# highreso-gpu/k8s-watcher

Measured on AMD Instinct MI355X. Metric: pod-events/sec sustained + p50 event→notify latency (single process, mock API), higher is better.
Workload: dtype n/a; 1 GPU; global_batch=1600000, parallelism=single-process (cluster watch), api_server=http, clusterapi=http, namespaces=64, target_namespaces=32, engine=native, validate=payload, state_format=structured

## Files before the change

### k8s_watcher_amd/ops/csrc/check/chunked_check.cpp

```cpp

#include <algorithm>
#include <cstdint>
#include <cstdio>
#include <cstdlib>
#include <cstring>
#include <fstream>
#include <iostream>
#include <memory>
#include <string>
#include <string_view>
#include <vector>

#if defined(__x86_64__)
#include <immintrin.h>
#endif

namespace {

#include "../scanner.inc"
#include "../chunked.inc"

struct Out {
    std::vector<std::string> lines;
    std::string end;
    bool operator==(const Out& o) const { return lines == o.lines && end == o.end; }
};

bool blank(const char* b, size_t n) {
    for (size_t i = 0; i < n; ++i)
        if (!(b[i] == ' ' || b[i] == '\r' || b[i] == '\t' || b[i] == '\n')) return false;
    return true;
}

std::string final_state(const ChunkState& st, bool open) {
    if (st.done()) return "done";
    return "state " + std::to_string(st.cstate) + " remain " + std::to_string(st.cremain) + " open " +
           std::to_string((int)open);
}

bool keep(Out& out, const char* b, size_t n) {
    if (n && !blank(b, n)) out.lines.emplace_back(b, n);
    return true;
}
// ... 116 lines not shown
```

### k8s_watcher_amd/ops/csrc/chunked.inc

```

enum { CS_SIZE, CS_DATA, CS_DATA_END, CS_TRAILER, CS_DONE };

bool parse_chunk_size(const char* line, size_t n, size_t& size, bool lenient) {
    size_t v = 0;
    size_t i = 0;
    while (lenient && i < n && (line[i] == ' ' || line[i] == '\t')) ++i;
    size_t start = i;
    for (; i < n; ++i) {
        int h = hexval(line[i]);
        if (h < 0) break;
        if (v > (SIZE_MAX >> 4)) return false;
        v = (v << 4) | (size_t)h;
    }
    if (i == start) return false;
    while (i < n && (line[i] == ' ' || line[i] == '\t' || (lenient && line[i] == '\r'))) ++i;
    if (i < n && line[i] != ';') return false;
    size = v;
    return true;
}

bool parse_chunk_size(const std::string& line, size_t& size) {
    return parse_chunk_size(line.data(), line.size(), size, true);
}

struct ChunkState {
    int cstate = CS_SIZE;
    size_t cremain = 0;
    std::string line;
    bool done() const { return cstate == CS_DONE; }
};

enum ChunkEnd {
    CE_MORE,
    CE_STOPPED,
    CE_DONE,
    CE_TOO_LONG,
    CE_BAD_SIZE,
};

constexpr size_t CHUNK_LINE_MAX = 4096;

std::string chunk_error_text(const ChunkState& st, ChunkEnd e) {
    if (e == CE_TOO_LONG) return "chunk size line too long";
    char msg[64];
    std::snprintf(msg, sizeof msg, "bad chunk size line %.40s", st.line.c_str());
    return msg;
}

template <class Sink>
inline ChunkEnd chunk_deframe(ChunkState& st, const char* base, size_t from, size_t to, size_t& at, Sink&& sink) {
    size_t i = from;
    ChunkEnd end = CE_MORE;
    while (i < to && end == CE_MORE) {
        switch (st.cstate) {
            case CS_SIZE: {
                const char* nl = (const char*)std::memchr(base + i, '\n', to - i);
                if (!nl) {
                    st.line.append(base + i, to - i);
                    i = to;
                    if (st.line.size() > CHUNK_LINE_MAX) end = CE_TOO_LONG;
                    break;
                }
                st.line.append(base + i, (size_t)(nl - (base + i)));
                i = (size_t)(nl - base) + 1;
                size_t size;
                if (!parse_chunk_size(st.line, size)) {
                    end = CE_BAD_SIZE;
                    break;
                }
                st.line.clear();
                if (size == 0) {
                    st.cstate = CS_TRAILER;
                } else {
                    st.cremain = size;
                    st.cstate = CS_DATA;
                }
                break;
            }
            case CS_DATA: {
                const size_t take = st.cremain < to - i ? st.cremain : to - i;
                if (!sink(i, take)) end = CE_STOPPED;
                i += take;
                st.cremain -= take;
                if (st.cremain == 0) st.cstate = CS_DATA_END;
                break;
            }
            case CS_DATA_END: {
                const char* nl = (const char*)std::memchr(base + i, '\n', to - i);
                if (!nl) {
                    i = to;
                    break;
                }
                i = (size_t)(nl - base) + 1;
                st.cstate = CS_SIZE;
                break;
            }
            case CS_TRAILER: {
                const char* nl = (const char*)std::memchr(base + i, '\n', to - i);
                if (!nl) {
                    st.line.append(base + i, to - i);
                    i = to;
                    break;
                }
                st.line.append(base + i, (size_t)(nl - (base + i)));
                i = (size_t)(nl - base) + 1;
                const bool empty = st.line.empty() || (st.line.size() == 1 && st.line[0] == '\r');
                st.line.clear();
                if (empty) {
                    st.cstate = CS_DONE;
                    end = CE_DONE;
                }
                break;
            }
            default:
                end = CE_DONE;
        }
    }
    at = i;
    return end;
}

enum : uint8_t {
    LN_WHOLE = 0,
    LN_FRAG = 1,
    LN_FRAG_END = 2,
};

template <class Sink>
inline bool split_lines(const char* base, size_t a, size_t n, bool& open, Sink&& sink) {
    size_t pos = a;
    const size_t end = a + n;
    while (pos < end) {
        const char* nl = (const char*)std::memchr(base + pos, '\n', end - pos);
        if (!nl) {
            open = true;
            return sink(LN_FRAG, pos, end - pos);
        }
        const size_t len = (size_t)(nl - base) - pos;
        const uint8_t kind = open ? LN_FRAG_END : LN_WHOLE;
        open = false;
        pos += len + 1;
        if (!sink(kind, pos - len - 1, len)) return false;
    }
    return true;
}

template <class Line>
inline bool join_line(std::string& partial, uint8_t kind, const char* b, size_t n, Line&& line) {
    if (kind == LN_WHOLE) return line(b, n, (std::string*)nullptr);
    partial.append(b, n);
    if (kind == LN_FRAG) return true;
    const bool go = line(partial.data(), partial.size(), &partial);
    partial.clear();
    return go;
}
```

### k8s_watcher_amd/ops/csrc/engine.inc

```


struct NReq {
    uint64_t seq = 0;
    std::string uid, etype, ns, name, body;
    size_t nbytes = 0;
    int64_t read_ns = 0, sent_ns = 0;
    int64_t submit_ns = 0;
    int attempts = 0;
    int conn = 0;
};

struct NConn {
    int fd = -1;
    bool up = false;
    std::deque<uint64_t> queue, inflight;
    std::string out;
    size_t out_off = 0;
    std::string in;
    bool dirty = false;
    SSL* ssl = nullptr;
    bool handshaking = false;
    bool write_wants_read = false;
    struct Staged {
        const char* p;
// ... 24 lines not shown
        ERR_error_string_n(e, buf, sizeof buf);
        msg += ": ";
        msg += buf;
    }
    ERR_clear_error();
    return msg;
}

int64_t mono_ns() {
    struct timespec ts;
    clock_gettime(CLOCK_MONOTONIC, &ts);
    return (int64_t)ts.tv_sec * 1000000000LL + ts.tv_nsec;
}

struct Probe {
    bool on = false;
    int64_t t0_ns = 0;
    uint64_t t0_tsc = 0;
    uint64_t calls = 0, lines = 0, bytes = 0, split = 0, wait = 0, apply = 0, run = 0, nio_calls = 0, nio = 0;
    uint64_t pump = 0;
    uint64_t tail = 0;
    uint64_t partitioned = 0;
    uint64_t tail_serial = 0;
    uint64_t tail_sent = 0, tail_submit = 0;
    uint64_t tail_rv = 0;
    long double age_byte_ns = 0;
};
Probe g_probe;

struct ApplyStats {
    std::atomic<uint64_t> par_batches{0}, par_lines{0}, tail_serial{0}, tail_submits{0}, tail_lock_runs{0};
    std::atomic<uint64_t> serial_batches{0}, serial_lines{0};
    std::atomic<uint64_t> payload_built{0}, payload_prefiltered{0};
};
ApplyStats g_apply;

uint32_t crc32_bytes(const char* p, size_t n) {
    return (uint32_t)::crc32(0L, reinterpret_cast<const Bytef*>(p), (uInt)n);
}

struct NotifierCore {
    std::recursive_mutex mu;
    bool threaded = false;
    int ep = -1, wake_fd = -1, py_fd = -1;
    std::thread io;
    std::atomic<bool> io_quit{false};
    std::vector<uint8_t> epout;
    int64_t signal_below = -1;
    int64_t signal_below_bytes = -1;

    std::vector<NConn> conns;
    using ReqMap = std::unordered_map<uint64_t, NReq>;
    ReqMap reqs;
    SvMap<uint64_t> latest;
    SvMap<uint64_t> unsent;
    std::vector<ReqMap::node_type> free_reqs;
    std::vector<SvMap<uint64_t>::node_type> free_latest;
    static constexpr size_t FREE_NODES_MAX = 4096;
    std::string head;
    int depth = 1;
    int max_attempts = 3;
    double delay = 2.0, multiplier = 2.0, max_delay = 30.0;
    bool coalesce = false, log_events = false;
    LogSink* sink = nullptr;
    std::vector<int> retryable;
    uint64_t next_seq = 0;
// ... 1422 lines not shown
    const std::string* env_json;
    int extra = 0;
    uint8_t validate = VALIDATE_PAYLOAD;
    const std::string* tz_utc = nullptr;
    bool failures = false;
    const ReasonSet* reasons = nullptr;
    bool conditions = false;
    const CondRules* rules = nullptr;
};

enum : uint8_t {
    JOB_FULL = 0,
    JOB_FIELDS = 1,
    JOB_PAYLOAD = 2,
    JOB_SKIP = 3,
};

struct ApplyHot {
    Span uid, ns, name, rv, phase;
    size_t uid_h = 0, ns_h = 0;
    const char* err = nullptr;
    const char* payload_err = nullptr;
    int tidx = -1;
    bool status_present = false, uid_hashed = false, ns_hashed = false;
    bool has_core = false, repr_fallback = false, obj_present = false;
    bool fail_cand = false;
    bool cond_cand = false;
    bool pre_dropped = false;
    uint8_t part = 255;
    uint8_t outcome = 0;
};

constexpr uint8_t PART_SERIAL = 255;

inline size_t none_uid_hash() {
    static const size_t h = sv_hash(NONE_UID);
    return h;
}

static_assert(sizeof(ApplyHot) <= 128, "ApplyHot is two cache lines");

struct alignas(64) LineJob {
    ApplyHot hot;
    const char* p = nullptr;
    size_t n = 0;
    PodSpans S;
    Span type_span, obj_span;
    const char* err = nullptr;
    const char* payload_err = nullptr;
    int tidx = -1;
    bool has_core = false;
    bool bare = false;
    bool repr_fallback = false;
    bool pre_dropped = false;
    uint8_t stage = 0;
    int64_t read_ns = 0;
    uint64_t fail_sig = 0;
    uint64_t cond_sig = 0;
    std::string core;
};

bool g_payload_prefilter = true;

inline bool payload_prefiltered(const DecodeCfg& C, const PodSpans& S) {
    std::string_view v;
    if (C.ns_texts && span_view(S.ns, v) && !C.ns_texts->has(v)) return true;
    if (C.shard_count > 1) {
        const Span& k = C.shard_by_uid ? S.uid : S.ns;
        v = std::string_view();
        if (!k.is_string() || span_view(k, v))
            return (int)(crc32_bytes(v.data(), v.size()) % (uint32_t)C.shard_count) != C.shard_index;
    }
    return false;
}

void decode_payload(const DecodeCfg& C, LineJob& J, bool prefilter = true) {
    PodSpans& S = J.S;
    const int tidx = J.tidx;
    J.pre_dropped = false;
    if (tidx < T_ADDED || tidx > T_DELETED || !J.obj_span.present()) return;
    static thread_local std::vector<Finding> found;
    const bool want_json = C.extra & EXTRA_FAILURES;
    J.fail_sig = 0;
    bool have_found = false;
    if ((C.failures && tidx != T_DELETED) || want_json) {
// ... 88 lines not shown
        P.object([&](const char* k, size_t kn) {
            if (KEYIS("type")) {
                J.type_span = P.value();
            } else if (KEYIS("object")) {
                S.clear();
                J.obj_span = Span();
                if (P.peek() != '{') {
                    P.value();
                    not_object = true;
                    return;
                }
                not_object = false;
                const char* start = P.p_;
                if (C.light) parse_pod_light(P, S); else parse_pod(P, S);
                J.obj_span.p = start;
                J.obj_span.n = (size_t)(P.p_ - start);
            } else {
                P.value();
            }
        });
        P.ws();
        if (P.p_ != P.end_) throw ParseError{"trailing data"};
        if (not_object) throw ParseError{"object is not a JSON object"};
        J.tidx = type_index(J.type_span);
    } catch (const ParseError& e) {
        J.err = e.msg;
        return;
    }
    if (J.stage == JOB_FIELDS) return;
    decode_payload(C, J);
}

void decode_line(const DecodeCfg& C, LineJob& J) {
    decode_line_impl(C, J);
    ApplyHot& H = J.hot;
    const PodSpans& S = J.S;
    H.uid = S.uid;
    H.ns = S.ns;
    H.name = S.name;
    H.rv = S.rv;
    H.phase = S.phase;
    H.status_present = S.status_present;
    H.err = J.err;
    H.payload_err = J.payload_err;
    H.tidx = J.tidx;
    H.has_core = J.has_core;
    H.repr_fallback = J.repr_fallback;
    H.pre_dropped = J.pre_dropped;
    H.fail_cand = J.fail_sig != 0;
    H.cond_cand = J.cond_sig != 0;
    H.obj_present = J.obj_span.present();
    std::string_view v;
    if ((H.uid_hashed = !J.err && span_view(S.uid, v))) H.uid_h = sv_hash(v);
    if ((H.ns_hashed = !J.err && span_view(S.ns, v))) H.ns_h = sv_hash(v);
    H.part = PART_SERIAL;
    H.outcome = 0;
    if (!J.err && J.tidx >= T_ADDED && J.tidx <= T_DELETED && H.obj_present) {
        if (!S.uid.is_string()) H.part = (uint8_t)PodStore::shard_of(none_uid_hash());
        else if (H.uid_hashed) H.part = (uint8_t)PodStore::shard_of(H.uid_h);
    }
}

long futex_call(std::atomic<uint32_t>* w, int op, uint32_t val) {
    return syscall(SYS_futex, reinterpret_cast<uint32_t*>(w), op, val, nullptr, nullptr, 0);
}

class DecodePool {
  public:
// ... 103 lines not shown
    void finish(uint32_t n) {
        while (done_.load(std::memory_order_acquire) < n)
            if (!work_one()) _mm_pause();
    }

  private:
    static constexpr uint32_t CLOSED = 0xFFFFFFFFu;
    static constexpr uint64_t APPLY_CLOSED = ~0ULL;
    static constexpr uint32_t GRAIN = 2;

    bool claim_part(uint32_t& g, uint32_t& p) {
        uint64_t c = apply_cur_.load(std::memory_order_acquire);
        while (true) {
            if (c == APPLY_CLOSED) return false;
            const uint32_t next = (uint32_t)(c & 0xFFFF), parts = (uint32_t)((c >> 16) & 0xFFFF);
            if (next >= parts) return false;
            if (apply_cur_.compare_exchange_weak(c, c + 1, std::memory_order_acq_rel, std::memory_order_acquire)) {
                g = (uint32_t)(c >> 32);
                p = next;
                return true;
            }
        }
    }

    void walk(uint32_t g, uint32_t p) {
        const ApplyPhase* ap = apply_.load(std::memory_order_acquire);
        std::atomic<uint32_t>* ready = readyp_.load(std::memory_order_acquire);
        const uint8_t* part = partp_.load(std::memory_order_acquire);
        const uint32_t n = total_.load(std::memory_order_acquire);
        uint32_t i = 0;
        for (; i < n; ++i) {
            while (ready[i].load(std::memory_order_acquire) != g)
                if (!work_one()) _mm_pause();
            if (part[i] != p) continue;
            if (!ap->apply(ap->ctx, i)) break;
            if (ap->prog) ap->prog[p].v.store(i + 1, std::memory_order_release);
        }
        ap->stop[p] = i;
        if (ap->prog) ap->prog[p].v.store(DONE | i, std::memory_order_release);
        parts_done_.fetch_add(1, std::memory_order_acq_rel);
    }

    bool work_one() {
        uint32_t got;
        return work_one(got);
    }
    bool work_one(uint32_t& got) {
        got = 0;
        uint64_t c = cursor_.load(std::memory_order_acquire);
        while (true) {
            uint32_t idx = (uint32_t)c;
            if (idx == CLOSED) return false;
            const DecodeCfg* cfg = cfg_.load(std::memory_order_acquire);
            const DecodeCfg* const* cfgs = cfgs_.load(std::memory_order_acquire);
            LineJob* jobs = jobs_.load(std::memory_order_acquire);
            std::atomic<uint32_t>* ready = readyp_.load(std::memory_order_acquire);
            uint8_t* part = partp_.load(std::memory_order_acquire);
            uint32_t n = total_.load(std::memory_order_acquire);
            if (idx >= n) return false;
            uint32_t end = idx + GRAIN < n ? idx + GRAIN : n;
            uint64_t next = (c & 0xFFFFFFFF00000000ULL) | end;
            if (!cursor_.compare_exchange_weak(c, next, std::memory_order_acq_rel, std::memory_order_acquire))
                continue;
            const uint32_t g = (uint32_t)(c >> 32);
            for (uint32_t i = idx; i < end; ++i) {
                decode_line(cfgs ? *cfgs[i] : *cfg, jobs[i]);
// ... 488 lines not shown
        LogSink& L = *self->sink->sink;
        if (self->log_events) {
            std::lock_guard<std::mutex> g(L.mu);
            L.begin(20);
            L.add("Pod event detected: ");
            L.add(k_type_name[S.tidx]);
            L.add(" - ", 3);
            who(L);
            L.end();
        }
        if (skipped && self->log_debug) {
            std::lock_guard<std::mutex> g(L.mu);
            L.begin(10);
            L.add("Skipping pod ");
            who(L);
            L.add(" - not in target namespaces");
            L.end();
        }
        return;
    }
    if (!self->log_events && !(skipped && self->log_debug)) return;
    PyObject* nso = span_to_str(S.ns);
    PyObject* nmo = span_to_str(S.name);
    const bool ok = nso && nmo;
    if (self->log_events)
        pl_log(self, 20, ok ? PyUnicode_FromFormat("Pod event detected: %s - %S/%S", k_type_name[S.tidx], nso, nmo)
                            : nullptr);
    if (skipped && self->log_debug)
        pl_log(self, 10, ok ? PyUnicode_FromFormat("Skipping pod %S/%S - not in target namespaces", nso, nmo) : nullptr);
    Py_XDECREF(nso);
    Py_XDECREF(nmo);
}

void apply_line(PipelineObject* self, LineJob& J) {
    if (apply_control(self, J)) return;
    const ApplyHot& S = J.hot;
    if (!self->silent) ++self->c_recv;
    if (S.rv.is_string() && S.rv.n > 2 && !self->relist_gen) self->rv_span = S.rv;
    std::string ns_buf, name_buf, rv_buf, phase_buf;
    LineNames N;
    N.key = none_key();
    if (S.uid.is_string()) {
        const std::string_view uid = text_of(S.uid, *self->key);
        N.key = HashedView{uid, S.uid_hashed ? S.uid_h : sv_hash(uid)};
    }
    N.ns = text_of(S.ns, ns_buf);
    if (self->shard_count > 1 && other_shard(self, S, N)) {
        apply_tally(self, OUT_SHARD);
        return;
    }
    N.name = text_of(S.name, name_buf);
    N.rv = text_of(S.rv, rv_buf);
    PodCacheObject* cache = self->cache;
    if (S.ns.is_string()) N.ns_id = cache->ns->intern(HashedView{N.ns, S.ns_h}, S.ns_hashed);
    if (S.status_present && S.phase.is_string()) N.phase_id = cache->phases->intern(text_of(S.phase, phase_buf));
    PodStore& store = *cache->store;
    const auto it = store.find(N.key);
    uint8_t out = self->silent ? OUT_NONE
                               : apply_verdict(self, J, N.ns_id, N.phase_id, it != store.end() ? &it->second : nullptr);
    if (out > OUT_CRIT && (self->log_events || self->log_debug)) log_line(self, S, N, out);
    if (out >= OUT_SENT && !line_core(self, J)) out = OUT_NONE;
    apply_commit(self, J, N, it, out);
    apply_tally(self, out);
    if (out < OUT_SENT) return;
    if (self->notifier) {
        submit_line(self, J, N);
        return;
// ... 24 lines not shown
    if (S.ns.is_string() && !S.ns_hashed) return false;
    LineNames N = plain_names(S);
    if (S.rv.is_string()) N.rv = str_body(S.rv);
    if (self->shard_count > 1 && other_shard(self, S, N)) {
        S.outcome = OUT_SHARD;
        return true;
    }
    PodCacheObject* cache = self->cache;
    if (S.ns.is_string() && (N.ns_id = cache->ns->lookup(HashedView{N.ns, S.ns_h}, true)) == UINT32_MAX) return false;
    if (S.status_present && S.phase.is_string() &&
        (N.phase_id = cache->phases->lookup(HashedView{str_body(S.phase), 0}, false)) == UINT32_MAX)
        return false;
    PodStore& store = *cache->store;
    const auto it = store.find(N.key);
    const uint8_t out = apply_verdict(self, J, N.ns_id, N.phase_id, it != store.end() ? &it->second : nullptr);
    if (out >= OUT_SENT && !S.has_core) return false;
    apply_commit(self, J, N, it, out);
    S.outcome = out;
    return true;
}

struct ParCtx {
    LineJob* jobs;
    PipelineObject* const* owner;
    PipelineObject* self;
    uint32_t stop[PodStore::SHARDS];
};

bool par_apply_one(void* c, uint32_t i) {
    ParCtx& x = *static_cast<ParCtx*>(c);
    return apply_par(x.owner ? x.owner[i] : x.self, x.jobs[i]);
}

struct PayloadTally {
    uint64_t built = 0, prefiltered = 0;
    void see(const ApplyHot& H) {
        built += H.has_core;
        prefiltered += H.pre_dropped;
    }
    void flush() {
        if (built) g_apply.payload_built.fetch_add(built, std::memory_order_relaxed);
        if (prefiltered) g_apply.payload_prefiltered.fetch_add(prefiltered, std::memory_order_relaxed);
        built = prefiltered = 0;
    }
};

bool g_partitioned_apply = true;
constexpr size_t PARTITION_MIN_LINES = 24;

bool partition_ok(PipelineObject* self, PipelineObject* const* owner, size_t nj) {
    if (!g_partitioned_apply || !self->pool || self->pool->size() == 0 || nj < PARTITION_MIN_LINES) return false;
    PipelineObject* last = nullptr;
    for (size_t i = 0; i < nj; ++i) {
        PipelineObject* pl = owner ? owner[i] : self;
        if (pl == last) continue;
        last = pl;
        if (!pl->notifier || pl->log_events || pl->log_debug || pl->relist_gen || pl->silent || pl->failed ||
            pl->cache != self->cache)
            return false;
        if (!owner) break;
    }
    return true;
}

void pl_push(PipelineObject* self, const char* b, size_t len) {
    if (!len || blank(b, len)) return;
    std::vector<LineJob>& v = *self->jobs_cur;
    if (self->njobs == v.size()) v.emplace_back();
    LineJob& J = v[self->njobs++];
    J.p = b;
    J.n = len;
    J.bare = false;
    J.stage = JOB_FULL;
    J.read_ns = self->read_ns;
}

inline void pl_piece(PipelineObject* self, uint8_t kind, const char* b, size_t n) {
    join_line(*self->partial, kind, b, n, [self](const char* lb, size_t ln, std::string* joined) {
        if (joined) {
            self->stitched->emplace_back(std::move(*joined));
            lb = self->stitched->back().data();
        }
        pl_push(self, lb, ln);
        return true;
    });
}

void pl_segment(PipelineObject* self, const char* data, size_t n) {
    bool open = !self->partial->empty();
    split_lines(data, 0, n, open, [&](uint8_t kind, size_t off, size_t len) {
        pl_piece(self, kind, data + off, len);
        return true;
    });
}

constexpr size_t PARALLEL_MIN_LINES = 6;
constexpr size_t PUMP_LINES = 1024;

inline void pl_pump(PipelineObject* self, size_t i) {
    if (!self->notifier) return;
    const NotifierCore& c = *self->notifier->core;
    const long long half = std::max<long long>(8, (long long)c.conns.size() * c.depth / 2);
    if (c.since_pump >= half || i % PUMP_LINES == PUMP_LINES - 1) {
        const uint64_t t0 = g_probe.on ? __rdtsc() : 0;
        {
// ... 9 lines not shown
    int depth = 0;
};
thread_local JobScratch tl_jobs;

struct ScratchGuard {
    PipelineObject* self;
    explicit ScratchGuard(PipelineObject* s) : self(s) {
        self->jobs_cur = tl_jobs.depth++ == 0 ? &tl_jobs.jobs : self->jobs;
    }
    ~ScratchGuard() { --tl_jobs.depth; }
};

PyObject* pl_run_impl(PipelineObject* self, const char* data, size_t len, long long read_ns, bool framed);

PyObject* pl_run(PipelineObject* self, PyObject* args, bool framed) {
    Py_buffer view;
    long long read_ns;
    int silent = 0;
    if (!PyArg_ParseTuple(args, "y*L|p", &view, &read_ns, &silent)) return nullptr;
    const bool was = self->silent;
    self->silent = was || silent;
    PyObject* res = pl_run_impl(self, (const char*)view.buf, (size_t)view.len, read_ns, framed);
    self->silent = was;
    PyBuffer_Release(&view);
    return res;
}

enum : uint8_t {
    HI_LINE = LN_WHOLE,
    HI_FRAG = LN_FRAG,
    HI_FRAG_END = LN_FRAG_END,
    HI_DONE = 3,
    HI_ERROR = 4,
};

struct HubItem {
    uint32_t off, len;
    uint8_t kind;
};

struct HubFrame {
    bool on = false;
    size_t upto = 0;
    std::vector<HubItem> items;
    std::string error;
};

bool pl_more(PipelineObject* self, const char* data, size_t len, long long read_ns, bool framed, PyObject* err[3]) {
    self->read_ns = read_ns;
    if (!framed) {
        pl_segment(self, data, len);
        return true;
    }
    if (self->failed) return true;
    size_t at;
    const ChunkEnd end = chunk_deframe(self->chunk, data, 0, len, at, [&](size_t off, size_t n) {
        pl_segment(self, data + off, n);
        return true;
    });
    if (end != CE_TOO_LONG && end != CE_BAD_SIZE) return true;
    set_chunk_error(self->chunk, end);
    PyErr_Fetch(&err[0], &err[1], &err[2]);
    return false;
}

bool pl_begin(PipelineObject* self, const char* data, size_t len, long long read_ns, bool framed, PyObject* err[3]) {
    self->ctrl = PyList_New(0);
    self->logs = nullptr;
    self->submits = nullptr;
    self->have_rv = false;
    self->rv_span = Span();
    self->ts->clear();
    self->c_recv = self->c_crit = self->c_ns = self->c_unch = self->c_shard = self->c_bm = self->c_fail = 0;
    self->c_cond = 0;
    self->read_ns = read_ns;
    self->failed = !self->ctrl;
    self->stitched->clear();
    err[0] = err[1] = err[2] = nullptr;
    return pl_more(self, data, len, read_ns, framed, err);
}

bool pl_items(PipelineObject* self, const char* data, const HubFrame& fr, long long read_ns, PyObject* err[3]);

bool pl_begin_items(PipelineObject* self, const char* data, const HubFrame& fr, long long read_ns, PyObject* err[3]) {
    pl_begin(self, data, 0, read_ns, false, err);
    return pl_items(self, data, fr, read_ns, err);
}

bool pl_items(PipelineObject* self, const char* data, const HubFrame& fr, long long read_ns, PyObject* err[3]) {
    self->read_ns = read_ns;
    for (const HubItem& it : fr.items) {
        switch (it.kind) {
            case HI_DONE:
                self->chunk.cstate = CS_DONE;
                break;
            case HI_ERROR:
                PyErr_SetString(PyExc_ValueError, fr.error.c_str());
                PyErr_Fetch(&err[0], &err[1], &err[2]);
                return false;
            default:
                pl_piece(self, it.kind, data + it.off, it.len);
        }
    }
    return true;
}

PyObject* pl_end(PipelineObject* self, bool ok, PyObject* err[3]) {
    if (self->rv_span.present()) {
        *self->last_rv = span_text(self->rv_span);
        self->have_rv = true;
        self->rv_known = true;
    }
    if (!ok) PyErr_Restore(err[0], err[1], err[2]);
    self->stitched->clear();
    PyObject* m = self->metrics;
    counter_add(m, "events_received", self->c_recv);
    counter_add(m, "events_filtered_critical", self->c_crit);
    counter_add(m, "events_filtered_namespace", self->c_ns);
    counter_add(m, "events_unchanged", self->c_unch);
    counter_add(m, "events_other_shard", self->c_shard);
    counter_add(m, "events_container_failure", self->c_fail);
    counter_add(m, "events_pod_condition", self->c_cond);
    counter_add(m, "bookmarks", self->c_bm);
    if (!ok || self->failed) {
        Py_CLEAR(self->ctrl);
        Py_CLEAR(self->logs);
        Py_CLEAR(self->submits);
        if (!PyErr_Occurred()) PyErr_SetString(PyExc_RuntimeError, "native pipeline failure");
        return nullptr;
    }
    PyObject* rv = self->have_rv ? PyUnicode_DecodeUTF8(self->last_rv->data(), (Py_ssize_t)self->last_rv->size(),
                                                       "replace")
// ... 48 lines not shown
                if (!pool->help()) {
                    _mm_pause();
                    if ((++spins & 1023) == 0) between();
                }
            }
            if (probe) t_wait += __rdtsc() - w0;
        }
        return (v & DecodePool::DONE) ? i < (v & ~DecodePool::DONE) : true;
    };
    const uint64_t t1 = probe ? __rdtsc() : 0;
    constexpr size_t TAIL_PREFETCH = 6;
    thread_local uint64_t epoch = 0;
    ++epoch;
    size_t npl = 0;
    constexpr int TAIL_LOCK_RUN = 32;
    if (nt) nlk = std::unique_lock<std::recursive_mutex>(nt->core->mu, std::defer_lock);
    uint64_t n_par = 0, n_serial = 0, n_sub = 0, n_runs = 0;
    PayloadTally payloads;
    for (size_t i = 0; i < nj; ++i) {
        if (i + TAIL_PREFETCH < nj) {
            __builtin_prefetch(&jobs[i + TAIL_PREFETCH].hot);
            __builtin_prefetch(reinterpret_cast<const char*>(&jobs[i + TAIL_PREFETCH].hot) + 64);
        }
        LineJob& J = jobs[i];
        PipelineObject* pl = owner ? owner[i] : self;
        if (pl->tail_epoch != epoch) {
            pl->tail_epoch = epoch;
            ++npl;
        }
        if (!pool->ready((uint32_t)i)) pool->await((uint32_t)i);
        if (pl->failed) continue;
        payloads.see(J.hot);
        const uint8_t p = J.hot.part;
        if (p != PART_SERIAL && (all_done ? i < ctx.stop[p] : applied(p, (uint32_t)i))) {
            ++n_par;
            ++pl->c_recv;
            pl->rv_fixed = false;
            const uint8_t out = J.hot.outcome;
            apply_tally(pl, out);
            if (out >= OUT_SENT) {
                const uint64_t s0 = probe ? __rdtsc() : 0;
                ++n_sub;
                const bool in_run = nt && pl->notifier == nt;
                if (in_run && !nlk.owns_lock()) {
                    nlk.lock();
                    ++n_runs;
                }
                submit_line(pl, J, plain_names(J.hot));
                if (!in_run) {
                    pl_pump(pl, i);
                } else if (++run == TAIL_LOCK_RUN) {
                    run = 0;
                    nlk.unlock();
                    pl_pump(pl, i);
                }
                if (probe) {
                    g_probe.tail_submit += __rdtsc() - s0;
                    ++g_probe.tail_sent;
                }
            }
            continue;
        }
        pl->rv_fixed = false;
        ++n_serial;
        if (probe) ++g_probe.tail_serial;
        if (nlk.owns_lock()) {
            nlk.unlock();
// ... 474 lines not shown
     "set_pod_conditions(on, rules=None): watcher.alerts.pod_conditions / pod_condition_rules"},
    {"set_repr", (PyCFunction)Pipeline_set_repr, METH_VARARGS,
     "set_repr(tz_utc_repr, fallback): state_format python_repr (pyrepr.inc)"},
    {"feed_chunked", (PyCFunction)Pipeline_feed_chunked, METH_VARARGS,
     "feed_chunked(data, read_ns) -> (ctrl, last_rv, logs, submits, ts)"},
    {"feed", (PyCFunction)Pipeline_feed, METH_VARARGS, "feed(data, read_ns): unframed NDJSON"},
    {"reset", (PyCFunction)Pipeline_reset, METH_NOARGS, "drop partial line / chunk state"},
    {"body_done", (PyCFunction)Pipeline_body_done, METH_NOARGS, "terminating chunk seen"},
    {"last_rv", (PyCFunction)Pipeline_last_rv, METH_NOARGS, "newest resourceVersion seen, or None"},
    {"set_last_rv", (PyCFunction)Pipeline_set_last_rv, METH_O, "set_last_rv(rv | None)"},
    {"set_log", (PyCFunction)Pipeline_set_log, METH_VARARGS, "set_log(log_events, log_debug)"},
    {"set_log_sink", (PyCFunction)Pipeline_set_log_sink, METH_O, "set_log_sink(LogSink | None): lines written natively"},
    {"decode_threads", (PyCFunction)Pipeline_decode_threads, METH_NOARGS, "worker threads in the decode pool"},
    {nullptr, nullptr, 0, nullptr}};

PyTypeObject PipelineType = {PyVarObject_HEAD_INIT(nullptr, 0)};

PyObject* kw_set_partitioned_apply(PyObject*, PyObject* arg) {
    const int on = PyObject_IsTrue(arg);
    if (on < 0) return nullptr;
    const bool prev = g_partitioned_apply;
    g_partitioned_apply = on;
    return PyBool_FromLong(prev);
}

PyObject* kw_set_payload_prefilter(PyObject*, PyObject* arg) {
    const int on = PyObject_IsTrue(arg);
    if (on < 0) return nullptr;
    const bool prev = g_payload_prefilter;
    g_payload_prefilter = on;
    return PyBool_FromLong(prev);
}

PyObject* kw_apply_partition(PyObject*, PyObject* arg) {
    Py_ssize_t n;
    const char* u = PyUnicode_Check(arg) ? PyUnicode_AsUTF8AndSize(arg, &n) : nullptr;
    if (!u) {
        if (!PyErr_Occurred()) PyErr_SetString(PyExc_TypeError, "uid must be a str");
        return nullptr;
    }
    return PyLong_FromLong((long)PodStore::shard_of(sv_hash(std::string_view(u, (size_t)n))));
}

PyObject* kw_apply_stats(PyObject*, PyObject*) {
    auto v = [](const std::atomic<uint64_t>& a) { return (unsigned long long)a.load(std::memory_order_relaxed); };
    return Py_BuildValue("{s:K,s:K,s:K,s:K,s:K,s:K,s:K,s:K,s:K}", "partitioned_batches", v(g_apply.par_batches),
                         "partitioned_lines", v(g_apply.par_lines), "tail_serial_lines", v(g_apply.tail_serial),
                         "tail_submits", v(g_apply.tail_submits), "tail_lock_runs", v(g_apply.tail_lock_runs),
                         "serial_batches", v(g_apply.serial_batches), "serial_lines", v(g_apply.serial_lines),
                         "payload_built", v(g_apply.payload_built), "payload_prefiltered",
                         v(g_apply.payload_prefiltered));
}

PyObject* kw_probe(PyObject*, PyObject* arg) {
    const int on = PyObject_IsTrue(arg);
    if (on < 0) return nullptr;
    Probe& P = g_probe;
    const int64_t now = mono_ns();
    const uint64_t tsc = __rdtsc();
    PyObject* out;
    if (P.t0_ns && now > P.t0_ns) {
        const double per_ns = (double)(tsc - P.t0_tsc) / (double)(now - P.t0_ns);
        auto ns = [per_ns](uint64_t ticks) { return (long long)((double)ticks / per_ns); };
        out = Py_BuildValue("{s:L,s:K,s:K,s:K,s:L,s:L,s:L,s:L,s:K,s:L,s:d,s:L,s:L,s:K}", "wall_ns", (long long)(now - P.t0_ns),
                            "calls", (unsigned long long)P.calls, "lines", (unsigned long long)P.lines, "bytes",
                            (unsigned long long)P.bytes, "split_ns", ns(P.split), "wait_ns", ns(P.wait), "apply_ns",
                            ns(P.apply), "run_ns", ns(P.run), "notifier_io_calls", (unsigned long long)P.nio_calls,
                            "notifier_io_ns", ns(P.nio), "data_age_us",
                            P.bytes ? (double)(P.age_byte_ns / (long double)P.bytes) / 1e3 : 0.0,
                            "pump_ns", ns(P.pump), "tail_ns", ns(P.tail), "partitioned_batches",
                            (unsigned long long)P.partitioned);
        if (out) {
            PyObject* extra = Py_BuildValue("{s:K,s:K,s:L,s:L}", "tail_serial_lines", (unsigned long long)P.tail_serial,
                                            "tail_sent", (unsigned long long)P.tail_sent, "tail_submit_ns",
                                            ns(P.tail_submit), "tail_rv_ns", ns(P.tail_rv));
            if (!extra || PyDict_Update(out, extra) < 0) {
                Py_XDECREF(extra);
                Py_DECREF(out);
                return nullptr;
// ... 39 lines not shown
```

### k8s_watcher_amd/ops/csrc/kwcore.cpp

```cpp

#define PY_SSIZE_T_CLEAN
#include <Python.h>

#include <arpa/inet.h>
#include <fcntl.h>
#include <openssl/err.h>
#include <openssl/evp.h>
#include <openssl/hmac.h>
#include <openssl/pem.h>
#include <openssl/ssl.h>
#include <openssl/x509v3.h>

#include <linux/futex.h>
#include <malloc.h>
#include <netinet/in.h>
#include <netinet/tcp.h>
#include <poll.h>
#include <sys/epoll.h>
#include <sys/ioctl.h>
#include <sys/mman.h>
#include <sys/sendfile.h>
#include <sys/resource.h>
#include <sys/eventfd.h>
#include <sys/socket.h>
#include <sys/syscall.h>
#include <sys/types.h>
#include <unistd.h>
#include <zlib.h>

#include <algorithm>
#include <array>
#include <charconv>
#include <chrono>
#include <atomic>
#include <cctype>
#include <cerrno>
#include <cmath>
#include <cstdint>
#include <cstdlib>
#include <cstring>
#include <ctime>
#include <condition_variable>
#include <deque>
#include <functional>
#include <memory>
#include <mutex>
#include <string>
#include <thread>
#include <unordered_map>
#include <unordered_set>
#include <vector>

#if defined(__x86_64__)
#include <immintrin.h>
#endif

namespace {

#include "scanner.inc"
#include "chunked.inc"


inline void put(std::string& o, const char* s, size_t n) { o.append(s, n); }
inline void put(std::string& o, const char* lit) { o.append(lit); }
inline void raw_or_null(std::string& o, const Span& s) {
    if (s.present()) o.append(s.p, s.n); else o.append("null", 4);
}

bool is_digit(char c) { return c >= '0' && c <= '9'; }

bool falsy_token(const Span& s) {
    if (!s.present()) return true;
    const char* p = s.p;
    size_t n = s.n;
    if (n == 4 && std::memcmp(p, "null", 4) == 0) return true;
    if (n == 5 && std::memcmp(p, "false", 5) == 0) return true;
    if (n == 2 && std::memcmp(p, "\"\"", 2) == 0) return true;
    if (p[0] == '{' || p[0] == '[') {
        for (size_t i = 1; i + 1 < n; ++i) {
            char c = p[i];
            if (!(c == ' ' || c == '\n' || c == '\r' || c == '\t')) return false;
// ... 1423 lines not shown
    if (!PyArg_ParseTuple(args, "nn", &mmap_thr, &trim_thr)) return nullptr;
    if (mmap_thr <= 0 || trim_thr <= 0 || mmap_thr > (Py_ssize_t)(32 << 20) || trim_thr > ((Py_ssize_t)1 << 30)) {
        PyErr_SetString(PyExc_ValueError, "malloc_tune: thresholds out of range");
        return nullptr;
    }
    const int a = mallopt(M_MMAP_THRESHOLD, (int)mmap_thr);
    const int b = mallopt(M_TRIM_THRESHOLD, (int)trim_thr);
    return PyBool_FromLong(a == 1 && b == 1);
}

PyMethodDef module_methods[] = {
    {"malloc_tune", (PyCFunction)kw_malloc_tune, METH_VARARGS,
     "malloc_tune(mmap_threshold, trim_threshold) -> ok (glibc mallopt; fixes both, disabling their sliding)"},
    {"malloc_trim", (PyCFunction)kw_malloc_trim, METH_NOARGS, "malloc_trim() -> released (glibc malloc_trim(0), no GIL)"},
    {"malloc_arenas", (PyCFunction)kw_malloc_arenas, METH_NOARGS,
     "malloc_arenas() -> [(arena, free_bytes, system_bytes)] (glibc malloc_info per arena)"},
    {"malloc_info", (PyCFunction)kw_malloc_info, METH_NOARGS,
     "malloc_info() -> {in_use_bytes, free_bytes, arena_bytes, mmap_bytes} (glibc mallinfo2)"},
    {"json_invalid", (PyCFunction)kw_json_invalid, METH_O, "json_invalid(data) -> None | reason (json.loads semantics)"},
    {"bench_validate", (PyCFunction)kw_bench_validate, METH_VARARGS, "bench_validate(lines, repeat) -> (seconds, invalid)"},
    {"bench_parse", (PyCFunction)kw_bench_parse, METH_VARARGS, "bench_parse(data, mode=2, repeat=1)"},
    {"event_timestamp", (PyCFunction)kw_event_timestamp, METH_O, "event_timestamp(utc) -> str"},
    {"stamp_fields", (PyCFunction)kw_stamp_fields, METH_VARARGS,
     "stamp_fields(buf, rv_off, rvs, ndigits, uid_off, uid_text): fixture re-stamping (int64 arrays)"},
    {"cpu_features", (PyCFunction)kw_cpu_features, METH_NOARGS, "SIMD paths in use"},
    {"set_simd", (PyCFunction)kw_set_simd, METH_O, "enable/disable the AVX2 scanner"},
    {"apply_stats", (PyCFunction)kw_apply_stats, METH_NOARGS,
     "apply_stats() -> cumulative counts of the partitioned and serial apply paths"},
    {"probe", (PyCFunction)kw_probe, METH_O, "probe(enable) -> event-loop thread time in native calls since the last call"},
    {"set_partitioned_apply", (PyCFunction)kw_set_partitioned_apply, METH_O,
     "set_partitioned_apply(on) -> previous: batches' apply phase split by pod-cache shard over the decode pool"},
    {"set_payload_prefilter", (PyCFunction)kw_set_payload_prefilter, METH_O,
     "set_payload_prefilter(on) -> previous: decode builds no payload for events the namespace or shard filter drops"},
    {"apply_partition", (PyCFunction)kw_apply_partition, METH_O,
     "apply_partition(uid) -> which of the partitioned apply's partitions takes the pod's lines"},
    {nullptr, nullptr, 0, nullptr}};

PyModuleDef moddef = {PyModuleDef_HEAD_INIT, "_kwcore", "native watch-event decoder", -1, module_methods};

}

PyMODINIT_FUNC PyInit__kwcore(void) {
    DecoderType.tp_name = "_kwcore.StreamDecoder";
    DecoderType.tp_basicsize = sizeof(DecoderObject);
    DecoderType.tp_flags = Py_TPFLAGS_DEFAULT;
    DecoderType.tp_doc = "StreamDecoder(environment, state_format='structured')";
    DecoderType.tp_methods = Decoder_methods;
    DecoderType.tp_new = Decoder_new;
    DecoderType.tp_init = (initproc)Decoder_init;
    DecoderType.tp_dealloc = (destructor)Decoder_dealloc;
    if (PyType_Ready(&DecoderType) < 0) return nullptr;
    PyObject* m = PyModule_Create(&moddef);
    if (!m) return nullptr;
    Py_INCREF(&DecoderType);
    PyModule_AddObject(m, "StreamDecoder", (PyObject*)&DecoderType);
    ScannerType.tp_name = "_kwcore.ResponseScanner";
    ScannerType.tp_basicsize = sizeof(ScannerObject);
    ScannerType.tp_flags = Py_TPFLAGS_DEFAULT;
    ScannerType.tp_doc = "ResponseScanner(): incremental HTTP/1.1 response framing";
    ScannerType.tp_methods = Scanner_methods;
    ScannerType.tp_new = Scanner_new;
    ScannerType.tp_dealloc = (destructor)Scanner_dealloc;
    if (PyType_Ready(&ScannerType) < 0) return nullptr;
    Py_INCREF(&ScannerType);
    PyModule_AddObject(m, "ResponseScanner", (PyObject*)&ScannerType);
    if (register_engine(m) < 0 || register_podcache(m) < 0 || register_pipeline(m) < 0 || register_logsink(m) < 0 ||
// ... 21 lines not shown
```

### k8s_watcher_amd/ops/csrc/readerhub.inc

```

constexpr int HUB_CLASSES = 4;

struct HubEntry {
    int sid;
    int buf;
    size_t len;
    int64_t read_ns;
    int err;
};

struct HubFramer {
    bool on = false;
    bool stopped = false;
    bool in_line = false;
    ChunkState chunk;

    void frame(const char* base, size_t from, size_t to, HubFrame& f) {
        f.upto = to;
        if (stopped) return;
        auto item = [&f](uint8_t kind, size_t off, size_t len) {
            if (len || kind != HI_LINE) f.items.push_back(HubItem{(uint32_t)off, (uint32_t)len, kind});
            return true;
        };
        size_t at;
        const ChunkEnd end = chunk_deframe(chunk, base, from, to, at, [&](size_t off, size_t len) {
            return split_lines(base, off, len, in_line, item);
        });
        if (end == CE_MORE) return;
        stopped = true;
        if (end != CE_DONE) f.error = chunk_error_text(chunk, end);
        item(end == CE_DONE ? HI_DONE : HI_ERROR, at, 0);
    }
};

struct HubStream {
    int fd = -1;
    bool paused = false;
    uint32_t armed = 0;
    int open = -1;
    int held = 0;
    bool reading = false;
    bool removed = false;
    SSL* ssl = nullptr;
    int phase = 0;
    bool want_out = false;
    bool starved = false;
    int cls = HUB_CLASSES - 1;
    int reading_buf = -1;
    HubFramer framer;
    TlsSecrets* secrets = nullptr;
    std::unique_ptr<Tls13Rx> rx;
    size_t ring_counted = 0;
    std::string out;
    size_t out_off = 0;
    int64_t last_ns = 0;
    int reader = -1;
    int64_t off_since_ns = 0;
};
// ... 1776 lines not shown
```

### k8s_watcher_amd/ops/csrc/relist.inc

```

uint32_t g_relist_gen = 0;

uint32_t next_relist_gen() {
    if (++g_relist_gen == 0) ++g_relist_gen;
    return g_relist_gen;
}

enum { RL_START, RL_ITEMS_FIRST, RL_ITEMS, RL_DONE };

constexpr size_t RELIST_BATCH = 128;

struct RelistObject {
    PyObject_HEAD
    PipelineObject* pl;
    PyObject* body;
    Py_buffer view;
    const char* cur;
    const char* end;
    int state;
    std::string* page_rv;
    std::string* page_cont;
    bool have_rv, have_cont;
    uint32_t gen;
    bool silent;
// ... 260 lines not shown
    if (!PyArg_ParseTuple(args, "dL", &budget_us, &read_ns)) return false;
    budget_ns = budget_us <= 0 ? 0 : (int64_t)(budget_us * 1000.0);
    return true;
}

PyObject* Relist_step(RelistObject* self, PyObject* args) {
    int64_t budget;
    long long read_ns;
    if (!parse_budget(args, budget, read_ns)) return nullptr;
    if (!self->body) {
        PyErr_SetString(PyExc_RuntimeError, "Relist.step: no page");
        return nullptr;
    }
    const int64_t t0 = mono_ns();
    relist_call_begin(self, read_ns);
    PipelineObject* pl = self->pl;
    std::vector<LineJob>& jobs = *self->jobs;
    DecodeCfg cfg = *pl->cfg;
    cfg.light = true;
    DecodePool* pool = pl->pool;
    const char* perr = nullptr;
    PayloadTally payloads;
    while (!pl->failed && self->state != RL_DONE) {
        size_t nj = 0;
        try {
            const char* ip;
            size_t in;
            while (nj < RELIST_BATCH && relist_next_item(self, ip, in)) {
                if (nj == jobs.size()) jobs.emplace_back();
                LineJob& J = jobs[nj++];
                J.p = ip;
                J.n = in;
                J.bare = true;
                J.stage = JOB_FIELDS;
                J.read_ns = pl->read_ns;
            }
        } catch (const ParseError& e) {
            perr = e.msg;
            self->state = RL_DONE;
        }
        const bool par1 = pool && nj >= PARALLEL_MIN_LINES;
        if (par1) {
            pool->start(jobs.data(), (uint32_t)nj, &cfg);
            pool->finish((uint32_t)nj);
        }
        size_t changed = 0;
        for (size_t i = 0; i < nj; ++i) {
            if (!par1) decode_line(cfg, jobs[i]);
            relist_classify(self, jobs[i]);
            changed += jobs[i].stage == JOB_PAYLOAD;
        }
        if (pool && changed >= PARALLEL_MIN_LINES) {
            pool->start(jobs.data(), (uint32_t)nj, &cfg);
            for (size_t i = 0; i < nj && !pl->failed; ++i) {
                pool->await((uint32_t)i);
                payloads.see(jobs[i].hot);
                relist_apply_item(self, jobs[i]);
                pl_pump(pl, i);
            }
            pool->finish((uint32_t)nj);
        } else {
            for (size_t i = 0; i < nj && !pl->failed; ++i) {
                decode_line(cfg, jobs[i]);
                payloads.see(jobs[i].hot);
                relist_apply_item(self, jobs[i]);
                pl_pump(pl, i);
// ... 485 lines not shown
```

Before: 3.338 million pod-events/s.

## Frame whole chunks ending in a newline as one line without scanning

When an HTTP chunk arrives whole and ends with a newline while no line is open, it is pushed directly as one line job instead of being scanned by split_lines for line ends. Decode detects chunks that actually hold several lines, marks them with a barrier partition, and applies them serially by splitting them then. This is meant to remove the per-byte newline scan on the watch stream's hot path, since the API server typically sends one event per chunk. The cost is extra barrier handling in partitioned apply, a memchr in decode for chunk jobs, and a global switch plus a new checker.

```diff
diff --git a/k8s_watcher_amd/ops/csrc/check/chunk_lines_check.cpp b/k8s_watcher_amd/ops/csrc/check/chunk_lines_check.cpp
--- /dev/null
+++ b/k8s_watcher_amd/ops/csrc/check/chunk_lines_check.cpp
@@ -0,0 +1,215 @@
+
+#include "../kwcore.cpp"
+
+#include <fstream>
+namespace {
+
+struct Lines {
+    std::vector<std::string> lines;
+    size_t chunk_jobs = 0, multi_jobs = 0;
+    int bad = 0;
+};
+
+void take_job(const DecodeCfg& C, Lines& out, const char* b, size_t n, bool chunk) {
+    if (!n || blank(b, n)) return;
+    std::unique_ptr<char[]> own(new char[n]);
+    std::memcpy(own.get(), b, n);
+    LineJob J;
+    J.p = own.get();
+    J.n = n;
+    J.bare = false;
+    J.chunk = chunk;
+    J.stage = JOB_FULL;
+    decode_line(C, J);
+    const bool has_nl = std::memchr(own.get(), '\n', n) != nullptr;
+    const bool multi = J.hot.part == PART_BARRIER;
+    out.chunk_jobs += chunk;
+    out.multi_jobs += multi;
+    if (multi != (chunk && has_nl)) {
+        std::fprintf(stderr, "a job of %zu bytes: chunk %d, line end inside %d, marked several lines %d\n", n,
+                     (int)chunk, (int)has_nl, (int)multi);
+        ++out.bad;
+    }
+    if (multi && (!J.hot.err || J.hot.has_core || J.hot.obj_present)) {
+        std::fprintf(stderr, "a several-lines job names a resume point or a payload\n");
+        ++out.bad;
+    }
+    if (!chunk && has_nl) {
+        std::fprintf(stderr, "a scanned line holds a line end\n");
+        ++out.bad;
+    }
+    if (!multi) {
+        out.lines.emplace_back(own.get(), n);
+        return;
+    }
+    for (size_t pos = 0; pos < n;) {
+        const char* nl = (const char*)std::memchr(own.get() + pos, '\n', n - pos);
+        const size_t end = nl ? (size_t)(nl - own.get()) : n;
+        if (end > pos && !blank(own.get() + pos, end - pos)) {
+            LineJob sub;
+            sub.p = own.get() + pos;
+            sub.n = end - pos;
+            sub.stage = JOB_FULL;
+            decode_line(C, sub);
+            if (sub.hot.part == PART_BARRIER) {
+                std::fprintf(stderr, "a line of a several-lines job marked as several lines\n");
+                ++out.bad;
+            }
+            out.lines.emplace_back(sub.p, sub.n);
+        }
+        pos = end + 1;
+    }
+}
+
+Lines feed_pipeline(const DecodeCfg& C, const std::string& raw, size_t piece) {
+    Lines out;
+    ChunkState st;
+    std::string partial;
+    for (size_t lo = 0; lo < raw.size(); lo += piece) {
+        const size_t n = std::min(piece, raw.size() - lo);
+        std::unique_ptr<char[]> buf(new char[n]);
+        std::memcpy(buf.get(), raw.data() + lo, n);
+        const char* data = buf.get();
+        size_t at;
+        const ChunkEnd end = chunk_deframe(st, data, 0, n, at, [&](size_t off, size_t len, bool whole) {
+            if (chunk_is_line(data, off, len, whole, !partial.empty())) {
+                take_job(C, out, data + off, len - 1, true);
+                return true;
+            }
+            bool open = !partial.empty();
+            return split_lines(data, off, len, open, [&](uint8_t kind, size_t o, size_t ln) {
+                return join_line(partial, kind, data + o, ln, [&](const char* b, size_t bn, std::string*) {
+                    take_job(C, out, b, bn, false);
+                    return true;
+                });
+            });
+        });
+        if (end == CE_TOO_LONG || end == CE_BAD_SIZE) {
+            std::fprintf(stderr, "framing error: %s\n", chunk_error_text(st, end).c_str());
+            ++out.bad;
+            break;
+        }
+    }
+    if (!st.done() || !partial.empty()) {
+        std::fprintf(stderr, "the body did not end (state %d, %zu bytes of a line open)\n", st.cstate, partial.size());
+        ++out.bad;
+    }
+    return out;
+}
+
+Lines feed_hub(const DecodeCfg& C, const std::string& raw, size_t piece) {
+    constexpr size_t BUF = 256 * 1024;
+    Lines out;
+    HubFramer framer;
+    std::string partial;
+    bool done = false;
+    for (size_t base = 0; base < raw.size(); base += BUF) {
+        const size_t cap = std::min(BUF, raw.size() - base);
+        std::unique_ptr<char[]> buf(new char[cap]);
+        HubFrame f;
+        for (size_t len = 0; len < cap;) {
+            const size_t n = std::min(piece, cap - len);
+            std::memcpy(buf.get() + len, raw.data() + base + len, n);
+            len += n;
+            framer.frame(buf.get(), f.upto, len, f);
+        }
+        for (const HubItem& it : f.items) {
+            if (it.off > cap || it.len > cap - it.off) {
+                std::fprintf(stderr, "an item outside its buffer\n");
+                ++out.bad;
+                continue;
+            }
+            const char* b = buf.get() + it.off;
+            switch (it.kind) {
+                case HI_DONE: done = true; break;
+                case HI_ERROR:
+                    std::fprintf(stderr, "framing error: %s\n", f.error.c_str());
+                    ++out.bad;
+                    break;
+                case HI_CHUNK:
+                    if (!partial.empty()) {
+                        std::fprintf(stderr, "a chunk item while a line is open\n");
+                        ++out.bad;
+                    }
+                    take_job(C, out, b, it.len, true);
+                    break;
+                default:
+                    join_line(partial, it.kind, b, it.len, [&](const char* lb, size_t ln, std::string*) {
+                        take_job(C, out, lb, ln, false);
+                        return true;
+                    });
+            }
+        }
+    }
+    if (!done || !partial.empty()) {
+        std::fprintf(stderr, "the body did not end in the hub's framing\n");
+        ++out.bad;
+    }
+    return out;
+}
+
+}
+
+int main(int argc, char** argv) {
+    if (argc != 2) {
+        std::fprintf(stderr, "usage: %s CORPORA.tsv\n", argv[0]);
+        return 2;
+    }
+    std::ifstream in(argv[1]);
+    if (!in) {
+        std::fprintf(stderr, "cannot read %s\n", argv[1]);
+        return 2;
+    }
+    const std::string env_json = "\"production\"";
+    const ReasonSet reasons = default_failure_reasons();
+    const CondRules rules = default_condition_rules();
+    DecodeCfg C{};
+    C.light = true;
+    C.critical = true;
+    C.env_json = &env_json;
+    C.reasons = &reasons;
+    C.rules = &rules;
+
+    int total = 0;
+    std::string row;
+    while (std::getline(in, row)) {
+        const size_t tab = row.find('\t');
+        if (tab == std::string::npos) continue;
+        const std::string name = row.substr(0, tab);
+        std::string raw;
+        for (size_t i = tab + 1; i + 1 < row.size(); i += 2)
+            raw.push_back((char)((hexval(row[i]) << 4) | hexval(row[i + 1])));
+        g_chunk_lines = false;
+        const Lines want = feed_pipeline(C, raw, raw.size());
+        total += want.bad;
+        if (want.chunk_jobs || want.multi_jobs) {
+            std::fprintf(stderr, "%s: the switch is off, yet a chunk was taken unscanned\n", name.c_str());
+            ++total;
+        }
+        Lines shown;
+        for (const bool on : {true, false}) {
+            g_chunk_lines = on;
+            for (const size_t piece : {(size_t)1, (size_t)5000, (size_t)65536, raw.size()}) {
+                for (const bool hub : {false, true}) {
+                    const Lines got = hub ? feed_hub(C, raw, piece) : feed_pipeline(C, raw, piece);
+                    total += got.bad;
+                    if (got.lines != want.lines) {
+                        std::fprintf(stderr, "%s: switch %d, pieces of %zu, %s: %zu lines differ from the scanned %zu\n",
+                                     name.c_str(), (int)on, piece, hub ? "hub" : "pipeline", got.lines.size(),
+                                     want.lines.size());
+                        ++total;
+                    }
+                    if (!on && (got.chunk_jobs || got.multi_jobs)) {
+                        std::fprintf(stderr, "%s: the switch is off, yet a chunk was taken unscanned\n", name.c_str());
+                        ++total;
+                    }
+                    if (on && piece == raw.size() && !hub) shown = got;
+                }
+            }
+        }
+        g_chunk_lines = true;
+        std::printf("%s %zu %zu %zu\n", name.c_str(), shown.lines.size(), shown.chunk_jobs, shown.multi_jobs);
+    }
+    std::fprintf(stderr, "%d failures\n", total);
+    return total ? 1 : 0;
+}
diff --git a/k8s_watcher_amd/ops/csrc/check/chunked_check.cpp b/k8s_watcher_amd/ops/csrc/check/chunked_check.cpp
--- a/k8s_watcher_amd/ops/csrc/check/chunked_check.cpp
+++ b/k8s_watcher_amd/ops/csrc/check/chunked_check.cpp
@@ -9,6 +9,7 @@
 #include <memory>
 #include <string>
 #include <string_view>
+#include <type_traits>
 #include <vector>
 
 #if defined(__x86_64__)
diff --git a/k8s_watcher_amd/ops/csrc/chunked.inc b/k8s_watcher_amd/ops/csrc/chunked.inc
--- a/k8s_watcher_amd/ops/csrc/chunked.inc
+++ b/k8s_watcher_amd/ops/csrc/chunked.inc
@@ -51,6 +51,7 @@
 inline ChunkEnd chunk_deframe(ChunkState& st, const char* base, size_t from, size_t to, size_t& at, Sink&& sink) {
     size_t i = from;
     ChunkEnd end = CE_MORE;
+    bool fresh = false;
     while (i < to && end == CE_MORE) {
         switch (st.cstate) {
             case CS_SIZE: {
@@ -74,12 +75,19 @@
                 } else {
                     st.cremain = size;
                     st.cstate = CS_DATA;
+                    fresh = true;
                 }
                 break;
             }
             case CS_DATA: {
                 const size_t take = st.cremain < to - i ? st.cremain : to - i;
-                if (!sink(i, take)) end = CE_STOPPED;
+                bool go;
+                if constexpr (std::is_invocable_v<Sink&, size_t, size_t, bool>)
+                    go = sink(i, take, fresh && take == st.cremain);
+                else
+                    go = sink(i, take);
+                fresh = false;
+                if (!go) end = CE_STOPPED;
                 i += take;
                 st.cremain -= take;
                 if (st.cremain == 0) st.cstate = CS_DATA_END;
@@ -126,6 +134,12 @@
     LN_FRAG_END = 2,
 };
 
+bool g_chunk_lines = true;
+
+inline bool chunk_is_line(const char* base, size_t off, size_t len, bool whole, bool open) {
+    return whole && g_chunk_lines && !open && len > 1 && base[off + len - 1] == '\n';
+}
+
 template <class Sink>
 inline bool split_lines(const char* base, size_t a, size_t n, bool& open, Sink&& sink) {
     size_t pos = a;
diff --git a/k8s_watcher_amd/ops/csrc/engine.inc b/k8s_watcher_amd/ops/csrc/engine.inc
--- a/k8s_watcher_amd/ops/csrc/engine.inc
+++ b/k8s_watcher_amd/ops/csrc/engine.inc
@@ -80,6 +80,7 @@
     std::atomic<uint64_t> par_batches{0}, par_lines{0}, tail_serial{0}, tail_submits{0}, tail_lock_runs{0};
     std::atomic<uint64_t> serial_batches{0}, serial_lines{0};
     std::atomic<uint64_t> payload_built{0}, payload_prefiltered{0};
+    std::atomic<uint64_t> chunk_lines{0}, chunk_multi{0};
 };
 ApplyStats g_apply;
 
@@ -1568,6 +1569,7 @@
 };
 
 constexpr uint8_t PART_SERIAL = 255;
+constexpr uint8_t PART_BARRIER = 254;
 
 inline size_t none_uid_hash() {
     static const size_t h = sv_hash(NONE_UID);
@@ -1587,6 +1589,7 @@
     int tidx = -1;
     bool has_core = false;
     bool bare = false;
+    bool chunk = false;
     bool repr_fallback = false;
     bool pre_dropped = false;
     uint8_t stage = 0;
@@ -1741,8 +1744,17 @@
 }
 
 void decode_line(const DecodeCfg& C, LineJob& J) {
+    ApplyHot& H = J.hot;
+    if (J.chunk && !J.bare && J.stage == JOB_FULL && std::memchr(J.p, '\n', J.n)) {
+        J.err = J.payload_err = nullptr;
+        J.has_core = J.repr_fallback = J.pre_dropped = false;
+        J.tidx = -1;
+        H = ApplyHot();
+        H.err = "several lines in one chunk";
+        H.part = PART_BARRIER;
+        return;
+    }
     decode_line_impl(C, J);
-    ApplyHot& H = J.hot;
     const PodSpans& S = J.S;
     H.uid = S.uid;
     H.ns = S.ns;
@@ -1912,6 +1924,7 @@
         for (; i < n; ++i) {
             while (ready[i].load(std::memory_order_acquire) != g)
                 if (!work_one()) _mm_pause();
+            if (part[i] == PART_BARRIER) break;
             if (part[i] != p) continue;
             if (!ap->apply(ap->ctx, i)) break;
             if (ap->prog) ap->prog[p].v.store(i + 1, std::memory_order_release);
@@ -2466,7 +2479,55 @@
     Py_XDECREF(nmo);
 }
 
+void apply_line(PipelineObject* self, LineJob& J);
+bool blank(const char* b, size_t n);
+
+void apply_multi(PipelineObject* self, LineJob& J) {
+    thread_local LineJob tl_sub;
+    thread_local bool tl_sub_busy = false;
+    std::unique_ptr<LineJob> own;
+    if (tl_sub_busy) own.reset(new LineJob());
+    LineJob& sub = own ? *own : tl_sub;
+    const bool was_busy = tl_sub_busy;
+    tl_sub_busy = true;
+    uint64_t built = 0, prefiltered = 0;
+    ApplyHot last = J.hot;
+    const char* p = J.p;
+    const char* const e = J.p + J.n;
+    while (p < e && !self->failed) {
+        const char* nl = (const char*)std::memchr(p, '\n', (size_t)(e - p));
+        const char* le = nl ? nl : e;
+        if (le > p && !blank(p, (size_t)(le - p))) {
+            sub.p = p;
+            sub.n = (size_t)(le - p);
+            sub.bare = sub.chunk = false;
+            sub.stage = JOB_FULL;
+            sub.read_ns = J.read_ns;
+            decode_line(*self->cfg, sub);
+            const ApplyHot& H = sub.hot;
+            built += H.has_core;
+            prefiltered += H.pre_dropped;
+            if (!H.err && H.obj_present && H.rv.is_string() &&
+                (H.tidx == T_BOOKMARK ||
+                 (H.tidx >= T_ADDED && H.tidx <= T_DELETED && H.rv.n > 2 && !self->relist_gen))) {
+                last = H;
+                last.part = PART_BARRIER;
+            }
+            apply_line(self, sub);
+        }
+        p = nl ? nl + 1 : e;
+    }
+    tl_sub_busy = was_busy;
+    J.hot = last;
+    if (built) g_apply.payload_built.fetch_add(built, std::memory_order_relaxed);
+    if (prefiltered) g_apply.payload_prefiltered.fetch_add(prefiltered, std::memory_order_relaxed);
+}
+
 void apply_line(PipelineObject* self, LineJob& J) {
+    if (J.hot.part == PART_BARRIER) {
+        apply_multi(self, J);
+        return;
+    }
     if (apply_control(self, J)) return;
     const ApplyHot& S = J.hot;
     if (!self->silent) ++self->c_recv;
@@ -2557,13 +2618,20 @@
     return apply_par(x.owner ? x.owner[i] : x.self, x.jobs[i]);
 }
 
+thread_local uint64_t tl_chunk_jobs = 0;
+
 struct PayloadTally {
     uint64_t built = 0, prefiltered = 0;
+    uint64_t multi = 0;
     void see(const ApplyHot& H) {
         built += H.has_core;
         prefiltered += H.pre_dropped;
+        multi += H.part == PART_BARRIER;
     }
     void flush() {
+        if (tl_chunk_jobs) g_apply.chunk_lines.fetch_add(tl_chunk_jobs, std::memory_order_relaxed);
+        if (multi) g_apply.chunk_multi.fetch_add(multi, std::memory_order_relaxed);
+        tl_chunk_jobs = multi = 0;
         if (built) g_apply.payload_built.fetch_add(built, std::memory_order_relaxed);
         if (prefiltered) g_apply.payload_prefiltered.fetch_add(prefiltered, std::memory_order_relaxed);
         built = prefiltered = 0;
@@ -2588,7 +2656,7 @@
     return true;
 }
 
-void pl_push(PipelineObject* self, const char* b, size_t len) {
+void pl_push(PipelineObject* self, const char* b, size_t len, bool chunk = false) {
     if (!len || blank(b, len)) return;
     std::vector<LineJob>& v = *self->jobs_cur;
     if (self->njobs == v.size()) v.emplace_back();
@@ -2596,6 +2664,8 @@
     J.p = b;
     J.n = len;
     J.bare = false;
+    J.chunk = chunk;
+    tl_chunk_jobs += chunk;
     J.stage = JOB_FULL;
     J.read_ns = self->read_ns;
 }
@@ -2671,6 +2741,7 @@
     HI_FRAG_END = LN_FRAG_END,
     HI_DONE = 3,
     HI_ERROR = 4,
+    HI_CHUNK = 5,
 };
 
 struct HubItem {
@@ -2693,8 +2764,11 @@
     }
     if (self->failed) return true;
     size_t at;
-    const ChunkEnd end = chunk_deframe(self->chunk, data, 0, len, at, [&](size_t off, size_t n) {
-        pl_segment(self, data + off, n);
+    const ChunkEnd end = chunk_deframe(self->chunk, data, 0, len, at, [&](size_t off, size_t n, bool whole) {
+        if (chunk_is_line(data, off, n, whole, !self->partial->empty()))
+            pl_push(self, data + off, n - 1, true);
+        else
+            pl_segment(self, data + off, n);
         return true;
     });
     if (end != CE_TOO_LONG && end != CE_BAD_SIZE) return true;
@@ -2737,6 +2811,9 @@
                 PyErr_SetString(PyExc_ValueError, fr.error.c_str());
                 PyErr_Fetch(&err[0], &err[1], &err[2]);
                 return false;
+            case HI_CHUNK:
+                pl_push(self, data + it.off, it.len, true);
+                break;
             default:
                 pl_piece(self, it.kind, data + it.off, it.len);
         }
@@ -2851,7 +2928,7 @@
         if (pl->failed) continue;
         payloads.see(J.hot);
         const uint8_t p = J.hot.part;
-        if (p != PART_SERIAL && (all_done ? i < ctx.stop[p] : applied(p, (uint32_t)i))) {
+        if (p < PodStore::SHARDS && (all_done ? i < ctx.stop[p] : applied(p, (uint32_t)i))) {
             ++n_par;
             ++pl->c_recv;
             pl->rv_fixed = false;
@@ -3392,6 +3469,14 @@
     return PyBool_FromLong(prev);
 }
 
+PyObject* kw_set_chunk_lines(PyObject*, PyObject* arg) {
+    const int on = PyObject_IsTrue(arg);
+    if (on < 0) return nullptr;
+    const bool prev = g_chunk_lines;
+    g_chunk_lines = on;
+    return PyBool_FromLong(prev);
+}
+
 PyObject* kw_apply_partition(PyObject*, PyObject* arg) {
     Py_ssize_t n;
     const char* u = PyUnicode_Check(arg) ? PyUnicode_AsUTF8AndSize(arg, &n) : nullptr;
@@ -3404,7 +3489,8 @@
 
 PyObject* kw_apply_stats(PyObject*, PyObject*) {
     auto v = [](const std::atomic<uint64_t>& a) { return (unsigned long long)a.load(std::memory_order_relaxed); };
-    return Py_BuildValue("{s:K,s:K,s:K,s:K,s:K,s:K,s:K,s:K,s:K}", "partitioned_batches", v(g_apply.par_batches),
+    return Py_BuildValue("{s:K,s:K,s:K,s:K,s:K,s:K,s:K,s:K,s:K,s:K,s:K}", "chunk_lines", v(g_apply.chunk_lines),
+                         "chunk_multi", v(g_apply.chunk_multi), "partitioned_batches", v(g_apply.par_batches),
                          "partitioned_lines", v(g_apply.par_lines), "tail_serial_lines", v(g_apply.tail_serial),
                          "tail_submits", v(g_apply.tail_submits), "tail_lock_runs", v(g_apply.tail_lock_runs),
                          "serial_batches", v(g_apply.serial_batches), "serial_lines", v(g_apply.serial_lines),
diff --git a/k8s_watcher_amd/ops/csrc/kwcore.cpp b/k8s_watcher_amd/ops/csrc/kwcore.cpp
--- a/k8s_watcher_amd/ops/csrc/kwcore.cpp
+++ b/k8s_watcher_amd/ops/csrc/kwcore.cpp
@@ -47,6 +47,7 @@
 #include <mutex>
 #include <string>
 #include <thread>
+#include <type_traits>
 #include <unordered_map>
 #include <unordered_set>
 #include <vector>
@@ -1536,6 +1537,8 @@
      "set_partitioned_apply(on) -> previous: batches' apply phase split by pod-cache shard over the decode pool"},
     {"set_payload_prefilter", (PyCFunction)kw_set_payload_prefilter, METH_O,
      "set_payload_prefilter(on) -> previous: decode builds no payload for events the namespace or shard filter drops"},
+    {"set_chunk_lines", (PyCFunction)kw_set_chunk_lines, METH_O,
+     "set_chunk_lines(on) -> previous: a whole chunk that ends a line is framed as one line, unscanned"},
     {"apply_partition", (PyCFunction)kw_apply_partition, METH_O,
      "apply_partition(uid) -> which of the partitioned apply's partitions takes the pod's lines"},
     {nullptr, nullptr, 0, nullptr}};
diff --git a/k8s_watcher_amd/ops/csrc/readerhub.inc b/k8s_watcher_amd/ops/csrc/readerhub.inc
--- a/k8s_watcher_amd/ops/csrc/readerhub.inc
+++ b/k8s_watcher_amd/ops/csrc/readerhub.inc
@@ -23,7 +23,8 @@
             return true;
         };
         size_t at;
-        const ChunkEnd end = chunk_deframe(chunk, base, from, to, at, [&](size_t off, size_t len) {
+        const ChunkEnd end = chunk_deframe(chunk, base, from, to, at, [&](size_t off, size_t len, bool whole) {
+            if (chunk_is_line(base, off, len, whole, in_line)) return item(HI_CHUNK, off, len - 1);
             return split_lines(base, off, len, in_line, item);
         });
         if (end == CE_MORE) return;
diff --git a/k8s_watcher_amd/ops/csrc/relist.inc b/k8s_watcher_amd/ops/csrc/relist.inc
--- a/k8s_watcher_amd/ops/csrc/relist.inc
+++ b/k8s_watcher_amd/ops/csrc/relist.inc
@@ -316,6 +316,7 @@
                 J.p = ip;
                 J.n = in;
                 J.bare = true;
+                J.chunk = false;
                 J.stage = JOB_FIELDS;
                 J.read_ns = pl->read_ns;
             }
```

Result: no change. 3.407 million pod-events/s, median of 2 (+2.1%).
